# AvishaiBarnoy/genomics-lm

Measured on AMD Instinct MI355X. Metric: codon tokens/sec training step, 12L8H d512 seq1024, higher is better.
Workload: dtype bf16; 1 GPU; TinyGPT 12L8H d512 T1024 V68 train step; model=TinyGPT (genomics-lm src/codonlm), global_batch=32, seq_len=1024, micro_batch_per_gpu=32, parallelism=dp1, sep_mask=True

## Files before the change

### genomics-lm_amd/csrc/gemm.hip

```cpp
#include "common.h"
#include <algorithm>

struct GemmParams {
  int M, N, K, kchunk;
  const void* A; long long lda;
  const void* B; long long ldb;
  void* C; long long ldc; int c_dtype;
  int epi; float alpha;
  const float* bias;
  const float* resid; long long ldr;
  const void* aux; void* aux_out; long long ld_aux;
  uint32_t drop_seed, drop_thr; float drop_scale;
  float* ws; int split;
  int n_valid;
  const float* rope_cos; const float* rope_sin;
  int rope_T, rope_half, rope_G, rope_mul, rope_uqk;
};

__device__ __forceinline__ void epi_apply(const GemmParams& p, int row, int col, float v) {
  const int e = p.epi;
  if (e & CG_EPI_BIAS) v += p.bias[col];
  const long long ai = (long long)row * p.ld_aux + col;
  if (e & CG_EPI_GELU) {
    const float s = (e & CG_EPI_GELU_DERIV) ? dgelu_f(v) : v;
// ... 269 lines not shown
template <bool KC>
__device__ __forceinline__ v8bf frag(const char* img, int rr0, int ks, int lane) {
  if (KC) {
    const int row = rr0 + (lane & 15), ch = ks * 4 + (lane >> 4);
    return *(const v8bf*)(img + kc_off(row, ch));
  } else {
    const int g = lane >> 4, i16 = lane & 15, q = i16 >> 2, pp = i16 & 3;
    const int krow = ks * 32 + 8 * g + q;
    const int ch = (rr0 >> 3) + (pp >> 1);
    const int b0 = mc_off(krow, ch) + 8 * (pp & 1);
    const int b1 = mc_off(krow + 4, ch) + 8 * (pp & 1);
    typedef v4s __attribute__((address_space(3))) * lp4;
    v4s lo = __builtin_amdgcn_ds_read_tr16_b64_v4i16((lp4)(img + b0));
    v4s hi = __builtin_amdgcn_ds_read_tr16_b64_v4i16((lp4)(img + b1));
    v8s r = {lo[0], lo[1], lo[2], lo[3], hi[0], hi[1], hi[2], hi[3]};
    return __builtin_bit_cast(v8bf, r);
  }
}
}

__device__ __forceinline__ void ld8f(const float* p, float v[8]) {
  const float4 a = *(const float4*)p, b = *(const float4*)(p + 4);
  v[0] = a.x; v[1] = a.y; v[2] = a.z; v[3] = a.w; v[4] = b.x; v[5] = b.y; v[6] = b.z; v[7] = b.w;
}
__device__ __forceinline__ void st8f(float* p, const float v[8]) {
  *(float4*)p = make_float4(v[0], v[1], v[2], v[3]);
  *(float4*)(p + 4) = make_float4(v[4], v[5], v[6], v[7]);
}
__device__ __forceinline__ void ld8b(const bf16_t* p, float v[8]) {
  const uint4 u = *(const uint4*)p;
  const uint32_t w[4] = {u.x, u.y, u.z, u.w};
#pragma unroll
  for (int j = 0; j < 4; ++j) {
    v[2 * j] = __uint_as_float(w[j] << 16);
    v[2 * j + 1] = __uint_as_float(w[j] & 0xFFFF0000u);
  }
}
__device__ __forceinline__ void st8b(bf16_t* p, const float v[8]) {
  uint4 u;
  u.x = (uint32_t)f2bf(v[0]) | ((uint32_t)f2bf(v[1]) << 16);
  u.y = (uint32_t)f2bf(v[2]) | ((uint32_t)f2bf(v[3]) << 16);
  u.z = (uint32_t)f2bf(v[4]) | ((uint32_t)f2bf(v[5]) << 16);
  u.w = (uint32_t)f2bf(v[6]) | ((uint32_t)f2bf(v[7]) << 16);
  *(uint4*)p = u;
}

template <int EPI, int CT>
__device__ __forceinline__ void epi_apply8(const GemmParams& p, int row, int col, float v[8]) {
  const int e = EPI >= 0 ? EPI : p.epi;
  const int ct = EPI >= 0 ? CT : p.c_dtype;
  if (e & CG_EPI_BIAS) {
    float bb[8];
    ld8f(p.bias + col, bb);
#pragma unroll
    for (int j = 0; j < 8; ++j) v[j] += bb[j];
  }
  const long long ai = (long long)row * p.ld_aux + col;
  if (e & CG_EPI_GELU) {
    if (e & CG_EPI_GELU_DERIV) {
      float dg[8];
#pragma unroll
      for (int j = 0; j < 8; ++j) v[j] = gelu_fast_d(v[j], dg[j]);
      if (ct == CG_BF16) st8b((bf16_t*)p.aux_out + ai, dg);
      else st8f((float*)p.aux_out + ai, dg);
    } else {
      if (ct == CG_BF16) st8b((bf16_t*)p.aux_out + ai, v);
      else st8f((float*)p.aux_out + ai, v);
#pragma unroll
      for (int j = 0; j < 8; ++j) v[j] = gelu_fast(v[j]);
    }
  }
  if (e & CG_EPI_DGELU) {
    float a[8];
    if (ct == CG_BF16) ld8b((const bf16_t*)p.aux + ai, a);
    else ld8f((const float*)p.aux + ai, a);
    if (e & CG_EPI_GELU_DERIV) {
#pragma unroll
      for (int j = 0; j < 8; ++j) v[j] *= a[j];
    } else {
#pragma unroll
      for (int j = 0; j < 8; ++j) v[j] *= dgelu_fast(a[j]);
    }
  }
  if (e & CG_EPI_DROPOUT) {
#pragma unroll
    for (int j = 0; j < 8; j += 2) {
      const uint32_t h = cg_hash_pair(p.drop_seed, (uint32_t)row, (uint32_t)(col + j) >> 1);
      v[j] = (h & 0xFFFFu) >= p.drop_thr ? v[j] * p.drop_scale : 0.f;
      v[j + 1] = (h >> 16) >= p.drop_thr ? v[j + 1] * p.drop_scale : 0.f;
    }
  }
  if (e & CG_EPI_RESID) {
    float r[8];
    ld8f(p.resid + (long long)row * p.ldr + col, r);
#pragma unroll
    for (int j = 0; j < 8; ++j) v[j] += r[j];
  }
  const long long ci = (long long)row * p.ldc + col;
  if (ct == CG_BF16) {
    st8b((bf16_t*)p.C + ci, v);
  } else {
    float* c = (float*)p.C + ci;
    if (e & CG_EPI_ACCUM) {
      float o[8];
      ld8f(c, o);
#pragma unroll
      for (int j = 0; j < 8; ++j) v[j] += o[j];
    }
    st8f(c, v);
  }
}

__global__ __launch_bounds__(256) void splitk_reduce_vec_kernel(GemmParams p) {
  const long long total8 = (long long)p.M * p.N / 8;
  const long long slab = (long long)p.M * p.N;
  for (long long i = blockIdx.x * 256ll + threadIdx.x; i < total8; i += (long long)gridDim.x * 256) {
    float s[8], t[8];
    ld8f(p.ws + i * 8, s);
    for (int z = 1; z < p.split; ++z) {
      ld8f(p.ws + z * slab + i * 8, t);
#pragma unroll
      for (int j = 0; j < 8; ++j) s[j] += t[j];
    }
    const long long e = i * 8;
    epi_apply8<-1, 0>(p, (int)(e / p.N), (int)(e % p.N), s);
  }
}

namespace bfg {
constexpr int EPI_LD = 68;
constexpr int EPI_BYTES = 4 * 64 * EPI_LD * 4;
constexpr int SMEM = EPI_BYTES > 4 * TILE_BYTES ? EPI_BYTES : 4 * TILE_BYTES;
}

template <bool AK, bool BKC, int EPI, int CT, bool VEC>
__device__ __forceinline__ void gemm_bf16_body(const GemmParams& p, char* smem) {
  using namespace bfg;
#define AS(i) (smem + (i) * TILE_BYTES)
#define BS(i) (smem + (2 + (i)) * TILE_BYTES)
  const int tid = threadIdx.x, wave = tid >> 6, lane = tid & 63;
  const int wm = (wave >> 1) * 64, wn = (wave & 1) * 64;
  const int nwg = gridDim.x * gridDim.y * gridDim.z;
  const int wg = cg_xcd_remap(blockIdx.x + gridDim.x * (blockIdx.y + gridDim.y * blockIdx.z), nwg);
  const int bz = wg / (gridDim.x * gridDim.y), bxy = wg % (gridDim.x * gridDim.y);
  const int m0 = (bxy / gridDim.x) * BM, n0 = (bxy % gridDim.x) * BN;
  const int kbeg = bz * p.kchunk;
  const int kend = min(p.K, kbeg + p.kchunk);
  const bf16_t* A = (const bf16_t*)p.A;
  const bf16_t* B = (const bf16_t*)p.B;

  v4f acc[4][4];
#pragma unroll
  for (int i = 0; i < 4; ++i)
#pragma unroll
    for (int j = 0; j < 4; ++j) acc[i][j] = (v4f){0.f, 0.f, 0.f, 0.f};

  const int nt = (kend - kbeg + BKT - 1) / BKT;
  Stage sa, sb;
  if (nt > 0) {
    stage_load<AK>(sa, A, p.lda, m0, p.M, kbeg, kend, tid);
    stage_load<BKC>(sb, B, p.ldb, n0, p.N, kbeg, kend, tid);
    stage_store<AK>(sa, AS(0), tid);
    stage_store<BKC>(sb, BS(0), tid);
  }
  __syncthreads();
  for (int t = 0; t < nt; ++t) {
    const int cur = t & 1;
    const bool more = (t + 1) < nt;
    if (more) {
      const int kn = kbeg + (t + 1) * BKT;
      stage_load<AK>(sa, A, p.lda, m0, p.M, kn, kend, tid);
      stage_load<BKC>(sb, B, p.ldb, n0, p.N, kn, kend, tid);
    }
#pragma unroll
    for (int ks = 0; ks < 2; ++ks) {
      v8bf af[4], bfr[4];
#pragma unroll
      for (int i = 0; i < 4; ++i) af[i] = frag<AK>(AS(cur), wm + 16 * i, ks, lane);
#pragma unroll
      for (int j = 0; j < 4; ++j) bfr[j] = frag<BKC>(BS(cur), wn + 16 * j, ks, lane);
      __builtin_amdgcn_s_setprio(1);
#pragma unroll
      for (int i = 0; i < 4; ++i)
#pragma unroll
        for (int j = 0; j < 4; ++j)
          acc[i][j] = __builtin_amdgcn_mfma_f32_16x16x32_bf16(af[i], bfr[j], acc[i][j], 0, 0, 0);
      __builtin_amdgcn_s_setprio(0);
    }
    if (more) {
      stage_store<AK>(sa, AS(cur ^ 1), tid);
      stage_store<BKC>(sb, BS(cur ^ 1), tid);
    }
    __syncthreads();
  }
#undef AS
#undef BS
  if (!VEC) {
#pragma unroll
    for (int i = 0; i < 4; ++i)
#pragma unroll
      for (int j = 0; j < 4; ++j)
#pragma unroll
        for (int v = 0; v < 4; ++v) {
          const int row = m0 + wm + 16 * i + 4 * (lane >> 4) + v;
          const int col = n0 + wn + 16 * j + (lane & 15);
          epi_store(p, row, col, acc[i][j][v], bz);
        }
    return;
  }
  float* st = (float*)smem + wave * 64 * EPI_LD;
#pragma unroll
  for (int i = 0; i < 4; ++i)
#pragma unroll
    for (int j = 0; j < 4; ++j)
#pragma unroll
      for (int v = 0; v < 4; ++v) st[(16 * i + 4 * (lane >> 4) + v) * EPI_LD + 16 * j + (lane & 15)] = acc[i][j][v];
  __syncthreads();
#pragma unroll 2
  for (int it = 0; it < 8; ++it) {
    const int c = lane + 64 * it, r = c >> 3, ch = c & 7;
    const int row = m0 + wm + r, col = n0 + wn + ch * 8;
    if (row >= p.M || col >= p.N) continue;
    float v[8];
    ld8f(st + r * EPI_LD + ch * 8, v);
#pragma unroll
    for (int j = 0; j < 8; ++j) v[j] *= p.alpha;
    if (p.split > 1) {
      st8f(p.ws + ((long long)bz * p.M + row) * p.N + col, v);
      continue;
    }
    epi_apply8<EPI, CT>(p, row, col, v);
  }
}

template <bool AK, bool BKC>
__global__ __launch_bounds__(256, 2) void gemm_bf16_kernel(GemmParams p) {
  extern __shared__ __attribute__((aligned(16))) char smem[];
  gemm_bf16_body<AK, BKC, -1, 0, false>(p, smem);
}

template <bool AK, bool BKC, int EPI, int CT>
__global__ __launch_bounds__(256, 2) void gemm_bf16_vec_kernel(GemmParams p) {
  extern __shared__ __attribute__((aligned(16))) char smem[];
  gemm_bf16_body<AK, BKC, EPI, CT, true>(p, smem);
}

#include "gemm_wide.h"
#include "gemm_pers.h"
#include "gemm_lw.h"
#include "gemm_dw.h"

__global__ __launch_bounds__(256) void colsum64_kernel(const void* C, long long ldc, int ct, int M, int N,
                                                       float* __restrict__ part) {
  const int n = blockIdx.x * 256 + threadIdx.x;
  if (n >= N) return;
  const int r0 = blockIdx.y * 64, r1 = min(M, r0 + 64);
  float acc = 0.f;
  for (int r = r0; r < r1; ++r)
    acc += ct == CG_BF16 ? bf2f(((const bf16_t*)C)[(long long)r * ldc + n]) : ((const float*)C)[(long long)r * ldc + n];
  part[(long long)blockIdx.y * N + n] = acc;
}

typedef void (*gemm_kernel_t)(GemmParams);

template <typename K>
static void launch4(K k00, K k01, K k10, K k11, bool ak, bool bk, dim3 g, dim3 b, size_t sh,
                    hipStream_t s, const GemmParams& p) {
  K k = ak ? (bk ? k11 : k10) : (bk ? k01 : k00);
  hipLaunchKernelGGL(k, g, b, sh, s, p);
}

template <template <bool, bool, int, int> class KS>
static gemm_kernel_t pick_spec(bool ak, bool bk, int e, int ct) {
#define SPEC(AK_, BK_, E, T) \
  if (ak == AK_ && bk == BK_ && e == (E) && ct == (T)) return KS<AK_, BK_, (E), (T)>::fn;
  SPEC(true, true, 0, CG_BF16)
  SPEC(true, true, 0, CG_F32)
  SPEC(true, true, CG_EPI_BIAS, CG_BF16)
  SPEC(true, true, CG_EPI_BIAS | CG_EPI_RESID, CG_F32)
  SPEC(true, true, CG_EPI_BIAS | CG_EPI_GELU, CG_BF16)
  SPEC(true, true, CG_EPI_BIAS | CG_EPI_DROPOUT | CG_EPI_RESID, CG_F32)
  SPEC(true, true, CG_EPI_RESID, CG_F32)
  SPEC(true, true, CG_EPI_DROPOUT | CG_EPI_RESID, CG_F32)
  SPEC(true, true, CG_EPI_DGELU, CG_BF16)
  SPEC(true, true, CG_EPI_BIAS | CG_EPI_GELU | CG_EPI_GELU_DERIV, CG_BF16)
  SPEC(true, true, CG_EPI_DGELU | CG_EPI_GELU_DERIV, CG_BF16)
  SPEC(true, false, 0, CG_BF16)
  SPEC(true, false, 0, CG_F32)
  SPEC(true, false, CG_EPI_DGELU, CG_BF16)
  SPEC(false, false, 0, CG_F32)
  SPEC(false, false, CG_EPI_ACCUM, CG_F32)
#undef SPEC
  if (ak) return bk ? KS<true, true, -1, 0>::fn : KS<true, false, -1, 0>::fn;
  return bk ? KS<false, true, -1, 0>::fn : KS<false, false, -1, 0>::fn;
}
template <bool AK, bool BKC, int E, int T>
struct VecK { static constexpr gemm_kernel_t fn = gemm_bf16_vec_kernel<AK, BKC, E, T>; };
template <bool AK, bool BKC, int E, int T>
struct WideK { static constexpr gemm_kernel_t fn = gemm_bf16_wide_kernel<AK, BKC, E, T>; };

static bool lw_auto_for(int e) {
  return e == 0 || e == CG_EPI_BIAS || e == (CG_EPI_BIAS | CG_EPI_GELU) ||
         e == (CG_EPI_BIAS | CG_EPI_GELU | CG_EPI_GELU_DERIV) || e == (CG_EPI_BIAS | CG_EPI_RESID) ||
         e == CG_EPI_RESID || e == CG_EPI_SWIGLU || (e & CG_EPI_ROPE);
}
static gemm_kernel_t pick_pers(int e, int ct, int tile, bool* lw_out) {
  bool lw = tile == CG_TILE_PERS_LW || (tile == CG_TILE_AUTO && lw_auto_for(e));
  if (e == CG_EPI_DSWIGLU) lw = false;
  if (e & CG_EPI_ROPE) {
    if (ct != CG_BF16 || !lw) return nullptr;
    *lw_out = true;
    if (e == (CG_EPI_BIAS | CG_EPI_ROPE)) return gemm_bf16_lw_kernel<CG_EPI_BIAS | CG_EPI_ROPE, CG_BF16>;
    if (e == CG_EPI_ROPE) return gemm_bf16_lw_kernel<CG_EPI_ROPE, CG_BF16>;
    return nullptr;
  }
  *lw_out = lw;
#define PSPEC(E, T) \
  if (e == (E) && ct == (T)) return lw ? gemm_bf16_lw_kernel<(E), (T)> : gemm_bf16_pers_kernel<(E), (T)>;
  PSPEC(0, CG_BF16)
  PSPEC(0, CG_F32)
  PSPEC(CG_EPI_BIAS, CG_BF16)
  PSPEC(CG_EPI_BIAS | CG_EPI_RESID, CG_F32)
  PSPEC(CG_EPI_BIAS | CG_EPI_GELU, CG_BF16)
  PSPEC(CG_EPI_BIAS | CG_EPI_DROPOUT | CG_EPI_RESID, CG_F32)
  PSPEC(CG_EPI_RESID, CG_F32)
  PSPEC(CG_EPI_DROPOUT | CG_EPI_RESID, CG_F32)
  PSPEC(CG_EPI_DGELU, CG_BF16)
  PSPEC(CG_EPI_ACCUM, CG_F32)
  PSPEC(CG_EPI_DGELU | CG_EPI_COLSUM, CG_BF16)
  PSPEC(CG_EPI_BIAS | CG_EPI_GELU | CG_EPI_GELU_DERIV, CG_BF16)
  PSPEC(CG_EPI_DGELU | CG_EPI_GELU_DERIV, CG_BF16)
  PSPEC(CG_EPI_DGELU | CG_EPI_GELU_DERIV | CG_EPI_COLSUM, CG_BF16)
  PSPEC(CG_EPI_COLSUM, CG_BF16)
  PSPEC(CG_EPI_SWIGLU, CG_BF16)
  PSPEC(CG_EPI_DSWIGLU, CG_BF16)
#undef PSPEC
  return nullptr;
}
static int cu_count() {
  static int n[64] = {0};
  int dev = 0;
  (void)hipGetDevice(&dev);
  if (dev < 0 || dev >= 64) dev = 0;
  if (!n[dev]) {
    int v = 0;
    if (hipDeviceGetAttribute(&v, hipDeviceAttributeMultiprocessorCount, dev) != hipSuccess || v <= 0) v = 256;
    n[dev] = v;
  }
  return n[dev];
}
extern "C" int cg_pers_cus(void) { return cu_count(); }
static bool use_pers(const cg_gemm_desc* d, int split) {
  if (split != 1) return false;
  if (d->tile != CG_TILE_AUTO && d->tile != CG_TILE_PERS && d->tile != CG_TILE_PERS_LW) return false;
  if (!d->a_kcontig || !d->b_kcontig) return false;
  if (d->K % bfp::BKT || d->K < 2 * bfp::BKT) return false;
  bool lw = false;
  if (!pick_pers(d->epilogue, d->c_dtype, d->tile, &lw)) return false;
  const long long lim = (long long)bfp::OOR - (1ll << 24);
  const long long es = d->c_dtype == CG_BF16 ? 2 : 4;
  if (((long long)(d->M - 1) * d->lda + d->K) * 2 >= lim) return false;
  if (((long long)(d->N - 1) * d->ldb + d->K) * 2 >= lim) return false;
  if (((long long)(d->M - 1) * d->ldc + d->N) * es >= lim) return false;
  if ((d->epilogue & CG_EPI_RESID) && ((long long)(d->M - 1) * d->ldr + d->N) * 4 >= lim) return false;
  if ((d->epilogue & (CG_EPI_GELU | CG_EPI_DGELU)) && ((long long)(d->M - 1) * d->ld_aux + d->N) * es >= lim)
    return false;
  if ((d->epilogue & (CG_EPI_SWIGLU | CG_EPI_DSWIGLU)) &&
      (((long long)(2 * d->N - 1) * d->ldb + d->K) * 2 >= lim ||
       ((long long)(d->M - 1) * d->ld_aux + 2 * d->N) * 2 >= lim ||
       ((long long)(d->M - 1) * d->ldc + 2 * d->N) * 2 >= lim))
    return false;
  return true;
}

static bool use_wide(const cg_gemm_desc* d, int kchunk, int split) {
  if (d->tile != CG_TILE_AUTO && d->tile != CG_TILE_WIDE) return false;
  if (d->K % bfw::BKT || kchunk % bfw::BKT || d->M < bfw::BM || d->N < bfw::BN) return false;
  if (d->tile == CG_TILE_WIDE) return true;
  if (!d->a_kcontig || !d->b_kcontig) return false;
  const long long tiles = (long long)cg_cdiv(d->M, bfw::BM) * cg_cdiv(d->N, bfw::BN) * split;
  return tiles >= 192;
}

static bool vec_ok(const cg_gemm_desc* d, int split) {
  const int e = d->epilogue;
  if (d->N % 8 || d->ldc % 8 || ((uintptr_t)d->C & 15)) return false;
  if ((e & CG_EPI_BIAS) && ((uintptr_t)d->bias & 15)) return false;
  if ((e & CG_EPI_RESID) && (d->ldr % 8 || ((uintptr_t)d->resid & 15))) return false;
  if ((e & (CG_EPI_GELU | CG_EPI_DGELU)) &&
      (d->ld_aux % 8 || ((uintptr_t)((e & CG_EPI_GELU) ? d->aux_out : d->aux) & 15)))
    return false;
  if (split > 1 && ((uintptr_t)d->workspace & 15)) return false;
  return true;
}

extern "C" int cg_gemm(const cg_gemm_desc* d, void* stream) {
  if (!d || d->M < 0 || d->N < 0 || d->K < 0) return CG_EINVAL;
  if (d->M == 0 || d->N == 0) return CG_OK;
  hipStream_t s = (hipStream_t)stream;
  GemmParams p{};
  p.M = d->M; p.N = d->N; p.K = d->K;
  p.A = d->A; p.lda = d->lda; p.B = d->B; p.ldb = d->ldb;
  p.C = d->C; p.ldc = d->ldc; p.c_dtype = d->c_dtype;
  p.epi = d->epilogue; p.alpha = d->alpha;
  p.bias = d->bias; p.resid = d->resid; p.ldr = d->ldr;
  p.aux = d->aux; p.aux_out = d->aux_out; p.ld_aux = d->ld_aux;
  p.drop_seed = d->drop_seed;
  p.drop_thr = cg_drop_threshold(d->drop_p);
  p.drop_scale = d->drop_p < 1.f ? 1.0f / (1.0f - d->drop_p) : 0.f;
  if ((p.epi & CG_EPI_ACCUM) && p.c_dtype != CG_F32) return CG_EINVAL;
  if ((p.epi & CG_EPI_BIAS) && !p.bias) return CG_EINVAL;
  if ((p.epi & CG_EPI_RESID) && !p.resid) return CG_EINVAL;
  if ((p.epi & CG_EPI_GELU) && !p.aux_out) return CG_EINVAL;
  if ((p.epi & CG_EPI_DGELU) && !p.aux) return CG_EINVAL;
  if ((p.epi & CG_EPI_GELU_DERIV) && !(p.epi & (CG_EPI_GELU | CG_EPI_DGELU))) return CG_EINVAL;
  if ((p.epi & CG_EPI_COLSUM) && (!d->workspace || d->split_k > 1)) return CG_EINVAL;
  if ((p.epi & CG_EPI_COLSUM) && d->ws_bytes < (size_t)cg_cdiv(p.M, 64) * (size_t)p.N * sizeof(float)) return CG_EINVAL;
  const bool swg = (p.epi & (CG_EPI_SWIGLU | CG_EPI_DSWIGLU)) != 0;
  if (swg) {
    if (p.epi != CG_EPI_SWIGLU && p.epi != CG_EPI_DSWIGLU) return CG_EUNSUPPORTED;
    if (d->in_dtype != CG_BF16 || p.c_dtype != CG_BF16 || d->split_k > 1 || !d->a_kcontig || !d->b_kcontig ||
        p.alpha != 1.0f || (p.N & 63) || (p.ldc & 7) || (p.ld_aux & 7) || ((uintptr_t)p.C & 15) ||
        ((uintptr_t)(p.epi == CG_EPI_SWIGLU ? p.aux_out : p.aux) & 15))
      return CG_EUNSUPPORTED;
    if (p.epi == CG_EPI_SWIGLU ? !p.aux_out : !p.aux) return CG_EINVAL;
    p.n_valid = d->n_valid > 0 ? std::min(d->n_valid, p.N) : p.N;
  }
  const bool rope = (p.epi & CG_EPI_ROPE) != 0;
  if (rope) {
    if ((p.epi & ~(CG_EPI_ROPE | CG_EPI_BIAS)) || !d->rope_cos || !d->rope_sin || d->rope_T <= 0) return CG_EINVAL;
    const int hd = d->rope_hd;
    if (d->in_dtype != CG_BF16 || p.c_dtype != CG_BF16 || d->split_k > 1 || hd <= 0 || hd % 16 ||
        d->rope_heads <= 0 || (long long)d->rope_heads * hd > p.N || p.N % 16 || p.N >= 65536 ||
        (((uintptr_t)d->rope_cos | (uintptr_t)d->rope_sin) & 15))
      return CG_EUNSUPPORTED;
    p.rope_cos = d->rope_cos;
    p.rope_sin = d->rope_sin;
    p.rope_T = d->rope_T;
    p.rope_half = hd / 2;
    p.rope_G = hd / 16;
    p.rope_mul = (65536 + p.rope_G - 1) / p.rope_G;
    p.rope_uqk = d->rope_heads * hd / 16;
  }
  if (d->tile < CG_TILE_AUTO || d->tile > CG_TILE_PERS_LW) return CG_EINVAL;
  if (d->tile != CG_TILE_AUTO && d->in_dtype != CG_BF16) return CG_EUNSUPPORTED;
  int split = d->split_k > 1 ? d->split_k : 1;
  const int bkt = d->in_dtype == CG_BF16 ? bfg::BKT : 16;
  if (d->K == 0) split = 1;
  int kchunk = cg_cdiv(cg_cdiv(d->K > 0 ? d->K : 1, split), bkt) * bkt;
  split = cg_cdiv(d->K > 0 ? d->K : 1, kchunk);
  if (split > 1 && (!d->workspace || d->ws_bytes < (size_t)split * (size_t)p.M * (size_t)p.N * sizeof(float)))
    return CG_EINVAL;
  p.kchunk = kchunk; p.split = split; p.ws = d->workspace;
  bool vec = false;
  const bool colsum = (p.epi & CG_EPI_COLSUM) != 0;
  bool colsum_fused = false;

  if (d->in_dtype == CG_F32) {
    p.epi &= ~CG_EPI_COLSUM;
    const bool big = !(d->lda & 3) && !(d->ldb & 3) && !((uintptr_t)d->A & 15) &&
                     !((uintptr_t)d->B & 15) && ((d->a_kcontig || d->b_kcontig) ? !(d->K & 3) : true) &&
                     (d->a_kcontig || !(d->M & 3)) && (d->b_kcontig || !(d->N & 3));
    if (big) {
      launch4(gemm_f32_big_kernel<false, false>, gemm_f32_big_kernel<false, true>, gemm_f32_big_kernel<true, false>,
              gemm_f32_big_kernel<true, true>, d->a_kcontig, d->b_kcontig,
              dim3(cg_cdiv(p.N, f32b::BN), cg_cdiv(p.M, f32b::BM), split), dim3(256), 0, s, p);
    } else {
      dim3 g(cg_cdiv(p.N, 64), cg_cdiv(p.M, 64), split);
      launch4(gemm_f32_kernel<false, false>, gemm_f32_kernel<false, true>, gemm_f32_kernel<true, false>,
              gemm_f32_kernel<true, true>, d->a_kcontig, d->b_kcontig, g, dim3(256), 0, s, p);
    }
  } else if (d->in_dtype == CG_BF16) {
    if ((d->lda & 7) || (d->ldb & 7)) return CG_EUNSUPPORTED;
    if (((uintptr_t)d->A & 15) || ((uintptr_t)d->B & 15)) return CG_EUNSUPPORTED;
    if (d->a_kcontig ? (d->K & 7) : (d->M & 7)) return CG_EUNSUPPORTED;
    if (d->b_kcontig ? (d->K & 7) : (d->N & 7)) return CG_EUNSUPPORTED;
    dim3 g(cg_cdiv(p.N, bfg::BN), cg_cdiv(p.M, bfg::BM), split);
    dim3 blk(256);
    size_t sh = bfg::SMEM;
    vec = vec_ok(d, split);
    gemm_kernel_t k;
    const bool pers = vec && use_pers(d, split);
    if ((swg || rope) && !pers) return CG_EUNSUPPORTED;
    if (!pers) p.epi &= ~CG_EPI_COLSUM;
    const int ke = split > 1 ? 0 : p.epi, kt = split > 1 ? CG_F32 : p.c_dtype;
    if (pers) {
      bool lw = false;
      k = pick_pers(p.epi, p.c_dtype, d->tile, &lw);
      colsum_fused = colsum;
      const int tiles = cg_cdiv(p.N, (p.epi & CG_EPI_SWIGLU) ? bfp::BN / 2 : bfp::BN) * cg_cdiv(p.M, bfp::BM);
      g = dim3(std::min(tiles, d->max_wg > 0 ? d->max_wg : cg_pers_cus()));
      blk = dim3(lw ? bfl::THREADS : bfp::THREADS);
      sh = lw ? bfl::SMEM : bfp::SMEM;
    } else if (vec && use_wide(d, kchunk, split)) {
      k = pick_spec<WideK>(d->a_kcontig, d->b_kcontig, ke, kt);
      g = dim3(cg_cdiv(p.N, bfw::BN) * cg_cdiv(p.M, bfw::BM) * split);
      blk = dim3(bfw::THREADS);
      sh = bfw::SMEM;
    } else if (vec && (d->tile == CG_TILE_AUTO || d->tile == CG_TILE_VEC)) {
      k = pick_spec<VecK>(d->a_kcontig, d->b_kcontig, ke, kt);
    } else if (d->tile != CG_TILE_AUTO && d->tile != CG_TILE_VEC) {
      return CG_EUNSUPPORTED;
    } else {
      k = d->a_kcontig ? (d->b_kcontig ? gemm_bf16_kernel<true, true> : gemm_bf16_kernel<true, false>)
                       : (d->b_kcontig ? gemm_bf16_kernel<false, true> : gemm_bf16_kernel<false, false>);
    }
    cg_func_lds((const void*)k, (int)sh);
    const int pk = pers ? CG_PROBE_GEMM_PERS
                        : d->a_kcontig ? (d->b_kcontig ? CG_PROBE_GEMM_FWD : CG_PROBE_GEMM_DX)
                                       : (d->b_kcontig ? CG_PROBE_NONE : CG_PROBE_GEMM_DW);
    cg_probe_begin(pk, s);
    hipLaunchKernelGGL(k, g, blk, sh, s, p);
    if (cg_probe_kind() == pk) {
      const double M = p.M, N = p.N, K = p.K, ce = p.c_dtype == CG_F32 ? 4.0 : 2.0;
      const bool sw = (p.epi & CG_EPI_SWIGLU) != 0, dsw = (p.epi & CG_EPI_DSWIGLU) != 0;
      const double nb = sw ? 2.0 * N : N;
      double bytes = 2.0 * (M * K + nb * K) + M * N * ce;
      if (p.epi & CG_EPI_BIAS) bytes += 4.0 * N;
      if (p.epi & CG_EPI_RESID) bytes += 4.0 * M * N;
      if (p.epi & (CG_EPI_GELU | CG_EPI_DGELU)) bytes += M * N * ce;
      if (p.epi & CG_EPI_ACCUM) bytes += 4.0 * M * N;
      if (sw) bytes += 2.0 * M * 2.0 * N;
      if (dsw) bytes += 2.0 * M * 2.0 * N + M * N * ce;
      if (p.epi & CG_EPI_COLSUM) bytes += 4.0 * cg_cdiv(p.M, 64) * N;
      cg_probe_end(pk, s, 2.0 * M * nb * K, bytes);
    }
  } else {
    return CG_EUNSUPPORTED;
  }
  CG_LAUNCH_CHECK();
  if (split > 1) {
    const long long total = (long long)p.M * p.N;
    if (vec) {
      int blocks = (int)((total / 8 + 255) / 256);
      if (blocks > 4096) blocks = 4096;
      hipLaunchKernelGGL(splitk_reduce_vec_kernel, dim3(blocks), dim3(256), 0, s, p);
    } else {
      int blocks = (int)((total + 255) / 256);
      if (blocks > 4096) blocks = 4096;
      hipLaunchKernelGGL(splitk_reduce_kernel, dim3(blocks), dim3(256), 0, s, p);
    }
    CG_LAUNCH_CHECK();
  }
  if (colsum && !colsum_fused) {
    hipLaunchKernelGGL(colsum64_kernel, dim3(cg_cdiv(p.N, 256), cg_cdiv(p.M, 64)), dim3(256), 0, s, p.C, p.ldc,
                       p.c_dtype, p.M, p.N, p.ws);
    CG_LAUNCH_CHECK();
  }
  return CG_OK;
}

#ifndef DW_RING_SLOTS
#define DW_RING_SLOTS 5
#endif
static bool dw_tile_code(int bm) { return bm == 128 || bm == 129 || bm == 256 || bm == 512; }
extern "C" int cg_gemm_dw_tiles(int bm, int N_out, int K_out) {
  if (!dw_tile_code(bm)) bm = 128;
  return cg_cdiv(N_out, bm >= 256 ? 256 : 128) * cg_cdiv(K_out, bm == 512 ? 256 : 128);
}
template <int BM, int NS, int BNT = bfd::BN, int BKT = DW_KUNIT>
static int launch_dw(bfd::Params& P, hipStream_t s) {
  using G = bfd::Geo<BM, NS, BNT, BKT>;
  bool cs = false;
  for (int i = 0; i < P.nprod; ++i) cs |= P.p[i].colsum != nullptr;
  auto kern = cs ? gemm_dw_kernel<BM, NS, BNT, true, BKT> : gemm_dw_kernel<BM, NS, BNT, false, BKT>;
  int ntiles = 0;
  for (int i = 0; i < P.nprod; ++i) {
    bfd::Prod& pr = P.p[i];
    pr.tiles_n = cg_cdiv(pr.K_out, BNT);
    pr.tile0 = ntiles;
    ntiles += cg_cdiv(pr.N_out, BM) * pr.tiles_n;
  }
  P.ntiles = ntiles * P.ksplit;
  if (!ntiles) return CG_OK;
  if (P.ksplit > 1) P.kc_steps = dw_kc_steps(P.K, P.ksplit);
  const int grid = std::min(P.ntiles, P.max_wg > 0 ? P.max_wg : cg_pers_cus());
  cg_func_lds((const void*)kern, G::SMEM);
  double flops = 0, bytes = 0;
  for (int i = 0; i < P.nprod; ++i) {
    const bfd::Prod& q = P.p[i];
    flops += 2.0 * q.N_out * (double)q.K_out * P.K;
    bytes += 2.0 * P.K * ((double)q.N_out + q.K_out) + (q.accum ? 8.0 : 4.0) * q.N_out * (double)q.K_out;
  }
  cg_probe_begin(CG_PROBE_GEMM_DW_GROUPED, s);
  hipLaunchKernelGGL(kern, dim3(grid), dim3(G::THREADS), G::SMEM, s, P);
  cg_probe_end(CG_PROBE_GEMM_DW_GROUPED, s, flops, bytes);
  if (P.ksplit > 1) {
    long long most = 0;
    double elems = 0;
    for (int i = 0; i < P.nprod; ++i) {
      most = std::max<long long>(most, (long long)P.p[i].N_out * P.p[i].K_out / 4);
      elems += (double)P.p[i].N_out * P.p[i].K_out;
    }
    cg_probe_begin(CG_PROBE_DW_SLAB, s);
    hipLaunchKernelGGL(dw_slab_reduce_kernel, dim3((unsigned)std::min<long long>(cg_cdiv(most, 256), 512), P.nprod),
                       dim3(256), 0, s, P);
    cg_probe_end(CG_PROBE_DW_SLAB, s, (P.ksplit - 1) * elems, (4.0 * (P.ksplit - 1) + 8.0) * elems);
  }
  CG_LAUNCH_CHECK();
  return CG_OK;
}
extern "C" size_t cg_gemm_dw_grouped_workspace(const cg_dw_group* grp) {
  if (!grp || grp->ksplit <= 1) return 0;
  size_t e = 0;
  for (int i = 0; i < grp->n && i < CG_DW_MAX; ++i)
    if (grp->p[i].N_out > 0 && grp->p[i].K_out > 0) e += (size_t)grp->p[i].N_out * (size_t)grp->p[i].K_out;
  return (size_t)(grp->ksplit - 1) * e * sizeof(float);
}
extern "C" size_t cg_gemm_dw_grouped_workspace(const cg_dw_group* grp);
extern "C" int cg_gemm_dw_grouped(const cg_dw_group* grp, void* stream) {
  if (!grp || grp->n < 0 || grp->n > CG_DW_MAX || grp->K <= 0) return CG_EINVAL;
  bfd::Params P{};
  P.nprod = 0;
  P.K = grp->K;
  const long long lim = (1ll << 31) - (1ll << 24);
  for (int i = 0; i < grp->n; ++i) {
    const cg_dw_product& q = grp->p[i];
    if (q.N_out <= 0 || q.K_out <= 0) continue;
    if (!q.A || !q.B || !q.C) return CG_EINVAL;
    if (q.N_out % 8 || q.K_out % 8 || q.lda % 8 || q.ldb % 8 || q.ldc % 4 || q.lda < q.N_out || q.ldb < q.K_out ||
        q.ldc < q.K_out)
      return CG_EUNSUPPORTED;
    if (((uintptr_t)q.A & 15) || ((uintptr_t)q.B & 15) || ((uintptr_t)q.C & 15)) return CG_EUNSUPPORTED;
    if (((long long)(grp->K - 1) * q.lda + q.N_out) * 2 >= lim || ((long long)(grp->K - 1) * q.ldb + q.K_out) * 2 >= lim)
      return CG_EUNSUPPORTED;
    bfd::Prod& pr = P.p[P.nprod++];
    pr.A = (const bf16_t*)q.A; pr.lda = q.lda;
    pr.B = (const bf16_t*)q.B; pr.ldb = q.ldb;
    pr.C = q.C; pr.ldc = q.ldc;
    pr.N_out = q.N_out; pr.K_out = q.K_out;
    pr.alpha = q.alpha; pr.accum = q.accumulate;
    pr.colsum = q.col_sum;
    if (q.col_sum && grp->ksplit > 1) return CG_EUNSUPPORTED;
  }
  if (!P.nprod) return CG_OK;
  P.ksplit = grp->ksplit > 1 ? grp->ksplit : 1;
  if (P.ksplit > 8) return CG_EUNSUPPORTED;
  if (P.ksplit > 1) {
    if (!grp->workspace || ((uintptr_t)grp->workspace & 15) || grp->ws_bytes < cg_gemm_dw_grouped_workspace(grp))
      return CG_EINVAL;
    P.slab = grp->workspace;
    long long off = 0;
    for (int i = 0; i < P.nprod; ++i) {
      P.slab_off[i] = off;
      off += (long long)P.p[i].N_out * P.p[i].K_out;
    }
    P.slab_stride = off;
  }
  hipStream_t s = (hipStream_t)stream;
  const int bm = grp->tile_m > 0 ? grp->tile_m : 128;
  P.max_wg = grp->max_wg;
  if (bm == 512) return launch_dw<256, DW_RING_SLOTS, 256, 32>(P, s);
  if (bm == 256) return launch_dw<256, 3>(P, s);
  if (bm == 129) return launch_dw<128, 5>(P, s);
  return launch_dw<128, 4>(P, s);
}
```

### genomics-lm_amd/csrc/gemm_lw.h

```cpp
namespace bfl {
constexpr int CWAVES = 8, LWAVES = 4, THREADS = 64 * (CWAVES + LWAVES);
constexpr int A_PIECES = bfw::A_BYTES / 1024, B_PIECES = bfw::B_BYTES / 1024;
constexpr int LA = A_PIECES / LWAVES, LB = B_PIECES / LWAVES;
constexpr int PER_STAGE = LA + LB;
constexpr int SMEM = bfp::SMEM;
}

template <int EPI, int CT>
__global__ __launch_bounds__(bfl::THREADS, 1) void gemm_bf16_lw_kernel(GemmParams p) {
  using namespace bfp;
  constexpr bool SWG = Epi<EPI, CT>::SWG, DSW = Epi<EPI, CT>::DSW;
  constexpr bool RP = (EPI & CG_EPI_ROPE) != 0;
  constexpr int BNO = SWG ? BN / 2 : BN;
  constexpr int ES = CT == CG_BF16 ? 2 : 4;
  auto rope_col = [&](int n) __attribute__((always_inline)) {
    const int U = ((n >> 6) << 2) | ((n >> 3) & 3), c = (n >> 5) & 1, e = n & 7;
    if (U < p.rope_uqk) {
      const int h = (U * p.rope_mul) >> 16;
      return h * 2 * p.rope_half + 8 * (U - h * p.rope_G) + c * p.rope_half + e;
    }
    return 16 * U + 8 * c + e;
  };
  extern __shared__ __attribute__((aligned(16))) char smem[];
  const int tid = threadIdx.x, lane = tid & 63;
  const int wave = __builtin_amdgcn_readfirstlane(tid >> 6);
  const int tiles_n = (p.N + BNO - 1) / BNO, tiles_m = (p.M + BM - 1) / BM;
  const int ntiles = tiles_n * tiles_m;
  const int nblk = gridDim.x;
  const int lb = cg_xcd_remap(blockIdx.x, nblk);
  const int my_tiles = lb < ntiles ? (ntiles - 1 - lb) / nblk + 1 : 0;
  const int nt = p.K / BKT;
  const int S = my_tiles * nt;
  auto tile_org = [&](int k, int& m0, int& n0) __attribute__((always_inline)) {
    const int tile = lb + k * nblk;
    m0 = (tile / tiles_n) * BM;
    n0 = (tile % tiles_n) * BNO;
  };

  if (wave >= bfl::CWAVES) {
    const int L = wave - bfl::CWAVES;
    const __amdgpu_buffer_rsrc_t ra = rsrc(p.A, ((long long)(p.M - 1) * p.lda + p.K) * 2);
    const __amdgpu_buffer_rsrc_t rb = rsrc(p.B, ((long long)((SWG ? 2 : 1) * p.N - 1) * p.ldb + p.K) * 2);
    uint32_t va[bfl::LA], vb[bfl::LB];
#pragma unroll
    for (int j = 0; j < bfl::LA; ++j) va[j] = bfw::src_off<true>((L + bfl::LWAVES * j) * 1024 + 16 * lane, p.lda);
#pragma unroll
    for (int j = 0; j < bfl::LB; ++j) {
      const int pos = (L + bfl::LWAVES * j) * 1024 + 16 * lane;
      vb[j] = SWG ? b_src_off_swg(pos, p.ldb, p.N) : b_src_off(pos, p.ldb);
    }
    uint32_t vcur[bfl::LB], vnext[bfl::LB];
    auto rope_offsets = [&](int k) __attribute__((always_inline)) {
      int m0, n0;
      tile_org(k < my_tiles ? k : 0, m0, n0);
#pragma unroll
      for (int j = 0; j < bfl::LB; ++j) {
        const int pos = (L + bfl::LWAVES * j) * 1024 + 16 * lane;
        const int row = pos >> 7, phys = (pos >> 4) & 7;
        vnext[j] = ((uint32_t)rope_col(n0 + row) * (uint32_t)p.ldb + 8u * (uint32_t)(phys ^ fb(row))) * 2u;
      }
    };
    auto issue = [&](int g) __attribute__((always_inline)) {
      uint32_t ao = OOR, bo = OOR;
      if (g < S) {
        const int k = g / nt, t = g - k * nt;
        int m0, n0;
        tile_org(k, m0, n0);
        ao = (uint32_t)(((long long)m0 * p.lda + t * BKT) * 2);
        if constexpr (RP) {
          bo = (uint32_t)(t * BKT * 2);
          if (t == 0) {
#pragma unroll
            for (int j = 0; j < bfl::LB; ++j) vcur[j] = vnext[j];
          }
        } else {
          bo = (uint32_t)(((long long)n0 * p.ldb + t * BKT) * 2);
        }
      }
      char* st = smem + (g % STAGES) * STAGE_BYTES;
#pragma unroll
      for (int j = 0; j < bfl::LA; ++j) bfw::dma16(ra, st + (L + bfl::LWAVES * j) * 1024, ao + va[j]);
#pragma unroll
      for (int j = 0; j < bfl::LB; ++j)
        bfw::dma16(rb, st + A_BYTES + (L + bfl::LWAVES * j) * 1024, RP ? (bo == OOR ? OOR : bo + vcur[j]) : bo + vb[j]);
      if constexpr (RP) {
        if ((g + 1) % nt == 0) rope_offsets((g + 1) / nt);
      }
    };
    if constexpr (RP) rope_offsets(0);
    issue(0);
    issue(1);
    for (int g = 0; g < S; ++g) {
      wait_vm<bfl::PER_STAGE>();
      __builtin_amdgcn_s_barrier();
      issue(g + 2);
    }
    asm volatile("s_waitcnt vmcnt(0)" ::: "memory");
    return;
  }

  const int wm = (wave >> 1) * 64, wn = (wave & 1) * 64;
  const __amdgpu_buffer_rsrc_t rc = rsrc(p.C, ((long long)(p.M - 1) * p.ldc + (DSW ? 2 : 1) * p.N) * ES);
  const int g4 = lane >> 4, r16 = lane & 15;
  u32x4 xa[4][2], xb[4][2], bq[2][2];
  auto cols_of = [&](int n0, int c) __attribute__((always_inline)) {
    if constexpr (RP) return rope_col(n0 + wn + 32 * c + 8 * g4);
    return SWG ? n0 + (wn >> 1) + 8 * g4 : n0 + wn + 32 * c + 8 * g4;
  };
  auto epi_loads = [&](int k, auto lo_t, auto hi_t, auto bias_t) __attribute__((always_inline)) {
    constexpr int LO = decltype(lo_t)::value, HI = decltype(hi_t)::value;
    int m0, n0;
    tile_org(k, m0, n0);
    if constexpr (decltype(bias_t)::value && (EPI & CG_EPI_BIAS) != 0) {
      const __amdgpu_buffer_rsrc_t rbias = rsrc(p.bias, (long long)p.N * 4);
#pragma unroll
      for (int c = 0; c < 2; ++c) {
        const int cc = cols_of(n0, c);
        const uint32_t o = cc < p.N ? (uint32_t)cc * 4u : OOR;
        bq[c][0] = bld(rbias, o);
        bq[c][1] = bld(rbias, o + 16);
      }
    }
#pragma unroll
    for (int i = LO; i < HI; ++i) {
      const int row = m0 + wm + 16 * i + r16;
      const bool rok = row < p.M;
#pragma unroll
      for (int c = 0; c < 2; ++c) {
        const int cc = cols_of(n0, c);
        const bool ok = rok && cc < p.N;
        if constexpr ((EPI & CG_EPI_RESID) != 0) {
          const __amdgpu_buffer_rsrc_t rr = rsrc(p.resid, ((long long)(p.M - 1) * p.ldr + p.N) * 4);
          const uint32_t o = ok ? (uint32_t)(((long long)row * p.ldr + cc) * 4) : OOR;
          xa[i][c] = bld(rr, o);
          xb[i][c] = bld(rr, o + 16);
        }
        if constexpr ((EPI & CG_EPI_DGELU) != 0) {
          const __amdgpu_buffer_rsrc_t rx = rsrc(p.aux, ((long long)(p.M - 1) * p.ld_aux + p.N) * ES);
          const uint32_t o = ok ? (uint32_t)(((long long)row * p.ld_aux + cc) * ES) : OOR;
          xa[i][c] = bld(rx, o);
          if constexpr (CT != CG_BF16) xb[i][c] = bld(rx, o + 16);
        }
        if constexpr ((EPI & CG_EPI_ACCUM) != 0) {
          const uint32_t o = ok ? (uint32_t)(((long long)row * p.ldc + cc) * ES) : OOR;
          xa[i][c] = bld(rc, o);
          xb[i][c] = bld(rc, o + 16);
        }
        if constexpr (DSW) {
          const __amdgpu_buffer_rsrc_t rx = rsrc(p.aux, ((long long)(p.M - 1) * p.ld_aux + 2 * p.N) * 2);
          const uint32_t o = ok ? (uint32_t)(((long long)row * p.ld_aux + cc) * 2) : OOR;
          xa[i][c] = bld(rx, o);
          xb[i][c] = bld(rx, ok ? o + (uint32_t)p.N * 2u : OOR);
        }
      }
    }
  };

  v4f acc[4][4];
  auto cstep = [&](int g) __attribute__((always_inline)) {
    asm volatile("s_waitcnt lgkmcnt(0)" ::: "memory");
    __builtin_amdgcn_s_barrier();
    __builtin_amdgcn_sched_barrier(0);
    const char* st = smem + (g % STAGES) * STAGE_BYTES;
    const char* as = st;
    const char* bs = st + A_BYTES;
    v8bf af[2][4], bfr[2][4];
#pragma unroll
    for (int i = 0; i < 4; ++i) af[0][i] = bfg::frag<true>(as, wm + 16 * i, 0, lane);
#pragma unroll
    for (int j = 0; j < 4; ++j) bfr[0][j] = bfrag(bs, wn, j, 0, lane);
#pragma unroll
    for (int gr = 0; gr < 8; ++gr) {
      const int i = gr >> 1, j0 = 2 * (gr & 1);
      acc[i][j0] = PMFMA(bfr[0][j0], af[0][i], acc[i][j0], 0, 0, 0);
      acc[i][j0 + 1] = PMFMA(bfr[0][j0 + 1], af[0][i], acc[i][j0 + 1], 0, 0, 0);
      if (gr < 4) af[1][gr] = bfg::frag<true>(as, wm + 16 * gr, 1, lane);
      else bfr[1][gr - 4] = bfrag(bs, wn, gr - 4, 1, lane);
    }
#pragma unroll
    for (int i = 0; i < 4; ++i)
#pragma unroll
      for (int j = 0; j < 4; ++j) acc[i][j] = PMFMA(bfr[1][j], af[1][i], acc[i][j], 0, 0, 0);
    __builtin_amdgcn_sched_group_barrier(0x100, 8, 0);
#pragma unroll
    for (int gr = 0; gr < 8; ++gr) {
      __builtin_amdgcn_sched_group_barrier(0x008, 2, 0);
      __builtin_amdgcn_sched_group_barrier(0x100, 1, 0);
    }
    __builtin_amdgcn_sched_group_barrier(0x008, 16, 0);
  };

  const bool scaled = p.alpha != 1.0f;
  auto epilogue = [&](int k) __attribute__((always_inline)) {
    int m0, n0;
    tile_org(k, m0, n0);
    if (__builtin_expect(scaled, 0)) {
      asm volatile("");
#pragma unroll
      for (int i = 0; i < 4; ++i)
#pragma unroll
        for (int j = 0; j < 4; ++j) acc[i][j] *= p.alpha;
    }
    int col[2];
    uint32_t off_c[4][2];
#pragma unroll
    for (int c = 0; c < 2; ++c) col[c] = cols_of(n0, c);
#pragma unroll
    for (int i = 0; i < 4; ++i) {
      const int row = m0 + wm + 16 * i + r16;
#pragma unroll
      for (int c = 0; c < 2; ++c)
        off_c[i][c] = (row < p.M && col[c] < p.N)
                          ? (uint32_t)(((long long)row * p.ldc + col[c]) * ES)
                          : OOR;
    }
    float bia[2][8];
    if constexpr ((EPI & CG_EPI_BIAS) != 0) {
#pragma unroll
      for (int c = 0; c < 2; ++c) unpack_f32(bq[c][0], bq[c][1], bia[c]);
    }
    float csum[2][8];
    if constexpr ((EPI & CG_EPI_COLSUM) != 0) {
#pragma unroll
      for (int c = 0; c < 2; ++c)
#pragma unroll
        for (int j = 0; j < 8; ++j) csum[c][j] = 0.f;
    }
    if constexpr (SWG) {
      const __amdgpu_buffer_rsrc_t rx = rsrc(p.aux_out, ((long long)(p.M - 1) * p.ld_aux + 2 * p.N) * 2);
#pragma unroll
      for (int i = 0; i < 4; ++i) {
        const int row = m0 + wm + 16 * i + r16;
        float g[8], u[8], sv[8];
#pragma unroll
        for (int h = 0; h < 2; ++h)
#pragma unroll
          for (int q = 0; q < 4; ++q) {
            g[4 * h + q] = acc[i][h][q];
            u[4 * h + q] = acc[i][2 + h][q];
          }
        const bool ok = off_c[i][0] != OOR;
        const uint32_t o = ok ? (uint32_t)(((long long)row * p.ld_aux + col[0]) * 2) : OOR;
        bst_aux(rx, o, pack_bf16(g));
        bst_aux(rx, ok ? o + (uint32_t)p.N * 2u : OOR, pack_bf16(u));
#pragma unroll
        for (int j = 0; j < 8; ++j) sv[j] = col[0] + j < p.n_valid ? silu_f(g[j]) * u[j] : 0.f;
        bst(rc, off_c[i][0], pack_bf16(sv));
      }
      return;
    } else if constexpr (DSW) {
#pragma unroll
      for (int i = 0; i < 4; ++i) {
#pragma unroll
        for (int c = 0; c < 2; ++c) {
          float v[8], g[8], u[8], dg[8], du[8];
#pragma unroll
          for (int h = 0; h < 2; ++h)
#pragma unroll
            for (int q = 0; q < 4; ++q) v[4 * h + q] = acc[i][2 * c + h][q];
          unpack_bf16(xa[i][c], g);
          unpack_bf16(xb[i][c], u);
#pragma unroll
          for (int j = 0; j < 8; ++j) {
            dg[j] = du[j] = 0.f;
            if (col[c] + j < p.n_valid) {
              const float sg = 1.0f / (1.0f + __expf(-g[j]));
              du[j] = v[j] * (g[j] * sg);
              dg[j] = v[j] * u[j] * sg * (1.0f + g[j] * (1.0f - sg));
            }
          }
          bst(rc, off_c[i][c], pack_bf16(dg));
          bst(rc, off_c[i][c] == OOR ? OOR : off_c[i][c] + (uint32_t)p.N * 2u, pack_bf16(du));
        }
      }
      return;
    } else if constexpr (RP) {
      const int U = (((n0 + wn) >> 6) << 2) | g4;
      const bool rot = U < p.rope_uqk;
      const int dim0 = rot ? 8 * (U - ((U * p.rope_mul) >> 16) * p.rope_G) : 0;
      const long long tab_bytes = (long long)p.rope_T * p.rope_half * 4;
      const __amdgpu_buffer_rsrc_t rcs = rsrc(p.rope_cos, tab_bytes), rsn = rsrc(p.rope_sin, tab_bytes);
      u32x4 cq[4][2], sq[4][2];
#pragma unroll
      for (int i = 0; i < 4; ++i) {
        const int row = m0 + wm + 16 * i + r16;
        const uint32_t t = (uint32_t)row % (uint32_t)p.rope_T;
        const uint32_t o = rot ? (t * (uint32_t)p.rope_half + (uint32_t)dim0) * 4u : OOR;
        cq[i][0] = bld(rcs, o);
        cq[i][1] = bld(rcs, o + 16);
        sq[i][0] = bld(rsn, o);
        sq[i][1] = bld(rsn, o + 16);
      }
#pragma unroll
      for (int i = 0; i < 4; ++i) {
        float v0[8], v1[8], cs[8], sn[8];
#pragma unroll
        for (int h = 0; h < 2; ++h)
#pragma unroll
          for (int u = 0; u < 4; ++u) {
            v0[4 * h + u] = acc[i][h][u];
            v1[4 * h + u] = acc[i][2 + h][u];
          }
        if constexpr ((EPI & CG_EPI_BIAS) != 0) {
#pragma unroll
          for (int j = 0; j < 8; ++j) {
            v0[j] += bia[0][j];
            v1[j] += bia[1][j];
          }
        }
        unpack_f32(cq[i][0], cq[i][1], cs);
        unpack_f32(sq[i][0], sq[i][1], sn);
#pragma unroll
        for (int j = 0; j < 8; ++j) {
          const float c = rot ? cs[j] : 1.0f;
          const float y0 = fmaf(v0[j], c, -v1[j] * sn[j]);
          const float y1 = fmaf(v1[j], c, v0[j] * sn[j]);
          v0[j] = y0;
          v1[j] = y1;
        }
        bst(rc, off_c[i][0], pack_bf16(v0));
        bst(rc, off_c[i][1], pack_bf16(v1));
      }
      return;
    }
#pragma unroll
    for (int i = 0; i < 4; ++i) {
      const int row = m0 + wm + 16 * i + r16;
#pragma unroll
      for (int c = 0; c < 2; ++c) {
        float v[8];
#pragma unroll
        for (int h = 0; h < 2; ++h)
#pragma unroll
          for (int u = 0; u < 4; ++u) v[4 * h + u] = acc[i][2 * c + h][u];
        if constexpr ((EPI & CG_EPI_BIAS) != 0) {
#pragma unroll
          for (int j = 0; j < 8; ++j) v[j] += bia[c][j];
        }
        if constexpr ((EPI & CG_EPI_GELU) != 0) {
          const __amdgpu_buffer_rsrc_t rx = rsrc(p.aux_out, ((long long)(p.M - 1) * p.ld_aux + p.N) * ES);
          const uint32_t o = off_c[i][c] == OOR ? OOR : (uint32_t)(((long long)row * p.ld_aux + col[c]) * ES);
          float s[8];
          if constexpr ((EPI & CG_EPI_GELU_DERIV) != 0) {
#pragma unroll
            for (int j = 0; j < 8; ++j) v[j] = gelu_fast_d(v[j], s[j]);
          } else {
#pragma unroll
            for (int j = 0; j < 8; ++j) s[j] = v[j];
          }
          if constexpr (CT == CG_BF16) {
            bst_aux(rx, o, pack_bf16(s));
          } else {
            bst(rx, o, (u32x4){__float_as_uint(s[0]), __float_as_uint(s[1]), __float_as_uint(s[2]), __float_as_uint(s[3])});
            bst(rx, o + 16, (u32x4){__float_as_uint(s[4]), __float_as_uint(s[5]), __float_as_uint(s[6]), __float_as_uint(s[7])});
          }
          if constexpr ((EPI & CG_EPI_GELU_DERIV) == 0) {
#pragma unroll
            for (int j = 0; j < 8; ++j) v[j] = gelu_fast(v[j]);
          }
        }
        if constexpr ((EPI & CG_EPI_DGELU) != 0) {
          float a[8];
          if constexpr (CT == CG_BF16) unpack_bf16(xa[i][c], a);
          else unpack_f32(xa[i][c], xb[i][c], a);
#pragma unroll
          for (int j = 0; j < 8; ++j) v[j] *= (EPI & CG_EPI_GELU_DERIV) ? a[j] : dgelu_fast(a[j]);
        }
        if constexpr ((EPI & CG_EPI_DROPOUT) != 0) {
          const uint32_t rh = cg_row_hash(p.drop_seed, (uint32_t)row);
#pragma unroll
          for (int j = 0; j < 8; j += 2) {
            const uint32_t hsh = cg_pair_mix(rh + ((uint32_t)(col[c] + j) >> 1) * CG_COLK);
            v[j] = (hsh & 0xFFFFu) >= p.drop_thr ? v[j] * p.drop_scale : 0.f;
            v[j + 1] = (hsh >> 16) >= p.drop_thr ? v[j + 1] * p.drop_scale : 0.f;
          }
        }
        if constexpr ((EPI & (CG_EPI_RESID | CG_EPI_ACCUM)) != 0) {
          float r[8];
          unpack_f32(xa[i][c], xb[i][c], r);
#pragma unroll
          for (int j = 0; j < 8; ++j) v[j] += r[j];
        }
        if constexpr ((EPI & CG_EPI_COLSUM) != 0) {
          const float keep = row < p.M ? 1.f : 0.f;
#pragma unroll
          for (int j = 0; j < 8; ++j) csum[c][j] = fmaf(keep, v[j], csum[c][j]);
        }
        if constexpr (CT == CG_BF16) {
          bst(rc, off_c[i][c], pack_bf16(v));
        } else {
          bst(rc, off_c[i][c], (u32x4){__float_as_uint(v[0]), __float_as_uint(v[1]), __float_as_uint(v[2]), __float_as_uint(v[3])});
          bst(rc, off_c[i][c] + 16, (u32x4){__float_as_uint(v[4]), __float_as_uint(v[5]), __float_as_uint(v[6]), __float_as_uint(v[7])});
        }
      }
    }
    if constexpr ((EPI & CG_EPI_COLSUM) != 0) {
#pragma unroll
      for (int c = 0; c < 2; ++c)
#pragma unroll
        for (int j = 0; j < 8; ++j) csum[c][j] = dpp_sum16(csum[c][j]);
      const int prow = (m0 + wm) >> 6;
      const __amdgpu_buffer_rsrc_t rw = rsrc(p.ws, (long long)((p.M + 63) >> 6) * p.N * 4);
#pragma unroll
      for (int c = 0; c < 2; ++c) {
        const uint32_t o = (r16 == 0 && col[c] < p.N) ? (uint32_t)(((long long)prow * p.N + col[c]) * 4) : OOR;
        bst(rw, o, (u32x4){__float_as_uint(csum[c][0]), __float_as_uint(csum[c][1]), __float_as_uint(csum[c][2]),
                           __float_as_uint(csum[c][3])});
        bst(rw, o + 16, (u32x4){__float_as_uint(csum[c][4]), __float_as_uint(csum[c][5]), __float_as_uint(csum[c][6]),
                                __float_as_uint(csum[c][7])});
      }
    }
  };

  constexpr int XW = ((EPI & CG_EPI_RESID) ? 2 : 0) + ((EPI & CG_EPI_DGELU) ? (CT == CG_BF16 ? 1 : 2) : 0) +
                     ((EPI & CG_EPI_ACCUM) ? 2 : 0) + (DSW ? 2 : 0);
  constexpr int HA0 = XW == 0 ? 4 : (32 - ((EPI & CG_EPI_BIAS) ? 16 : 0)) / (8 * XW);
  constexpr int HA = DSW ? 0 : (HA0 > 4 ? 4 : HA0);
  const int ta = nt >= 3 ? nt - 3 : 0;
  int g = 0;
  for (int k = 0; k < my_tiles; ++k) {
#pragma unroll
    for (int i = 0; i < 4; ++i)
#pragma unroll
      for (int j = 0; j < 4; ++j) acc[i][j] = (v4f){0.f, 0.f, 0.f, 0.f};
    for (int t = 0; t < nt; ++t, ++g) {
      cstep(g);
      if (t == ta) {
        __builtin_amdgcn_sched_barrier(0);
        epi_loads(k, std::integral_constant<int, 0>{}, std::integral_constant<int, HA>{}, std::true_type{});
      }
    }
    if constexpr (HA < 4)
      epi_loads(k, std::integral_constant<int, HA>{}, std::integral_constant<int, 4>{}, std::false_type{});
    asm volatile("s_waitcnt vmcnt(0)" ::: "memory");
    __builtin_amdgcn_sched_barrier(0);
    epilogue(k);
  }
}
```

Before: 2.301 million tokens/s.

## Prefetch next-stage LDS fragments mid-step in load-warp GEMM and retime epilogue loads

Restructures the compute-wave main loop of the load-warp persistent GEMM so the barrier and the first-half fragment reads for the next K stage happen in the middle of the current step's second-half MFMAs. This hides LDS read latency behind matrix work instead of stalling at the top of each step. It also changes where epilogue operand loads are issued (late for extra-input epilogues, bias last, halved for accumulate/colsum) to ease register pressure. Finally it routes bias+dropout+residual GEMMs to the LW kernel and allows single-K-tile GEMMs when that kernel is explicitly requested. Risks include higher register use and schedule changes across many epilogue variants.

```diff
diff --git a/genomics-lm_amd/csrc/gemm.hip b/genomics-lm_amd/csrc/gemm.hip
--- a/genomics-lm_amd/csrc/gemm.hip
+++ b/genomics-lm_amd/csrc/gemm.hip
@@ -595,7 +595,8 @@
 static bool lw_auto_for(int e) {
   return e == 0 || e == CG_EPI_BIAS || e == (CG_EPI_BIAS | CG_EPI_GELU) ||
          e == (CG_EPI_BIAS | CG_EPI_GELU | CG_EPI_GELU_DERIV) || e == (CG_EPI_BIAS | CG_EPI_RESID) ||
-         e == CG_EPI_RESID || e == CG_EPI_SWIGLU || (e & CG_EPI_ROPE);
+         e == CG_EPI_RESID || e == (CG_EPI_BIAS | CG_EPI_DROPOUT | CG_EPI_RESID) || e == CG_EPI_SWIGLU ||
+         (e & CG_EPI_ROPE);
 }
 static gemm_kernel_t pick_pers(int e, int ct, int tile, bool* lw_out) {
   bool lw = tile == CG_TILE_PERS_LW || (tile == CG_TILE_AUTO && lw_auto_for(e));
@@ -647,9 +648,10 @@
   if (split != 1) return false;
   if (d->tile != CG_TILE_AUTO && d->tile != CG_TILE_PERS && d->tile != CG_TILE_PERS_LW) return false;
   if (!d->a_kcontig || !d->b_kcontig) return false;
-  if (d->K % bfp::BKT || d->K < 2 * bfp::BKT) return false;
+  if (d->K % bfp::BKT || d->K < bfp::BKT) return false;
   bool lw = false;
   if (!pick_pers(d->epilogue, d->c_dtype, d->tile, &lw)) return false;
+  if (d->K < 2 * bfp::BKT && !(lw && d->tile == CG_TILE_PERS_LW)) return false;
   const long long lim = (long long)bfp::OOR - (1ll << 24);
   const long long es = d->c_dtype == CG_BF16 ? 2 : 4;
   if (((long long)(d->M - 1) * d->lda + d->K) * 2 >= lim) return false;
diff --git a/genomics-lm_amd/csrc/gemm_lw.h b/genomics-lm_amd/csrc/gemm_lw.h
--- a/genomics-lm_amd/csrc/gemm_lw.h
+++ b/genomics-lm_amd/csrc/gemm_lw.h
@@ -157,6 +157,74 @@
   };
 
   v4f acc[4][4];
+#ifndef CG_LW_NO_PREFETCH
+  constexpr int MR = 2;
+  v8bf af[2][4], bfr[2][4];
+  auto read_half0 = [&](int g) __attribute__((always_inline)) {
+    const char* st = smem + (g % STAGES) * STAGE_BYTES;
+#pragma unroll
+    for (int j = 0; j < 4; ++j) bfr[0][j] = bfrag(st + A_BYTES, wn, j, 0, lane);
+#pragma unroll
+    for (int i = 0; i < 4; ++i) af[0][i] = bfg::frag<true>(st, wm + 16 * i, 0, lane);
+  };
+  auto cstep = [&](int g, auto top_tag, auto mid_tag) __attribute__((always_inline)) {
+    constexpr bool MID = decltype(mid_tag)::value;
+    if constexpr (decltype(top_tag)::value) {
+      asm volatile("s_waitcnt lgkmcnt(0)" ::: "memory");
+      __builtin_amdgcn_s_barrier();
+      __builtin_amdgcn_sched_barrier(0);
+      read_half0(g);
+    }
+    const char* st = smem + (g % STAGES) * STAGE_BYTES;
+    const char* as = st;
+    const char* bs = st + A_BYTES;
+#pragma unroll
+    for (int gr = 0; gr < 8; ++gr) {
+      const int i = gr >> 1, j0 = 2 * (gr & 1);
+      acc[i][j0] = PMFMA(bfr[0][j0], af[0][i], acc[i][j0], 0, 0, 0);
+      acc[i][j0 + 1] = PMFMA(bfr[0][j0 + 1], af[0][i], acc[i][j0 + 1], 0, 0, 0);
+      if (gr < 4) af[1][gr] = bfg::frag<true>(as, wm + 16 * gr, 1, lane);
+      else bfr[1][gr - 4] = bfrag(bs, wn, gr - 4, 1, lane);
+    }
+    if constexpr (MID) {
+#pragma unroll
+      for (int i = 0; i < MR; ++i)
+#pragma unroll
+        for (int j = 0; j < 4; ++j) acc[i][j] = PMFMA(bfr[1][j], af[1][i], acc[i][j], 0, 0, 0);
+#pragma unroll
+      for (int gr = 0; gr < 8; ++gr) {
+        __builtin_amdgcn_sched_group_barrier(0x008, 2, 0);
+        __builtin_amdgcn_sched_group_barrier(0x100, 1, 0);
+      }
+      __builtin_amdgcn_sched_group_barrier(0x008, 4 * MR, 0);
+      __builtin_amdgcn_sched_barrier(0);
+      asm volatile("s_waitcnt lgkmcnt(0)" ::: "memory");
+      __builtin_amdgcn_s_barrier();
+      __builtin_amdgcn_sched_barrier(0);
+      read_half0(g + 1);
+#pragma unroll
+      for (int i = MR; i < 4; ++i)
+#pragma unroll
+        for (int j = 0; j < 4; ++j) acc[i][j] = PMFMA(bfr[1][j], af[1][i], acc[i][j], 0, 0, 0);
+#pragma unroll
+      for (int gr = 0; gr < 8; ++gr) {
+        __builtin_amdgcn_sched_group_barrier(0x100, 1, 0);
+        __builtin_amdgcn_sched_group_barrier(0x008, 1, 0);
+      }
+    } else {
+#pragma unroll
+      for (int i = 0; i < 4; ++i)
+#pragma unroll
+        for (int j = 0; j < 4; ++j) acc[i][j] = PMFMA(bfr[1][j], af[1][i], acc[i][j], 0, 0, 0);
+#pragma unroll
+      for (int gr = 0; gr < 8; ++gr) {
+        __builtin_amdgcn_sched_group_barrier(0x008, 2, 0);
+        __builtin_amdgcn_sched_group_barrier(0x100, 1, 0);
+      }
+      __builtin_amdgcn_sched_group_barrier(0x008, 16, 0);
+    }
+  };
+#else
   auto cstep = [&](int g) __attribute__((always_inline)) {
     asm volatile("s_waitcnt lgkmcnt(0)" ::: "memory");
     __builtin_amdgcn_s_barrier();
@@ -189,6 +257,7 @@
     }
     __builtin_amdgcn_sched_group_barrier(0x008, 16, 0);
   };
+#endif
 
   const bool scaled = p.alpha != 1.0f;
   auto epilogue = [&](int k) __attribute__((always_inline)) {
@@ -415,14 +484,45 @@
   constexpr int XW = ((EPI & CG_EPI_RESID) ? 2 : 0) + ((EPI & CG_EPI_DGELU) ? (CT == CG_BF16 ? 1 : 2) : 0) +
                      ((EPI & CG_EPI_ACCUM) ? 2 : 0) + (DSW ? 2 : 0);
   constexpr int HA0 = XW == 0 ? 4 : (32 - ((EPI & CG_EPI_BIAS) ? 16 : 0)) / (8 * XW);
+#ifndef CG_LW_NO_PREFETCH
+  constexpr int HA1 = DSW ? 0 : (HA0 > 4 ? 4 : HA0);
+  constexpr int HA = ((EPI & CG_EPI_ACCUM) || EPI == (CG_EPI_DGELU | CG_EPI_COLSUM)) ? HA1 / 2 : HA1;
+#else
   constexpr int HA = DSW ? 0 : (HA0 > 4 ? 4 : HA0);
+#endif
   const int ta = nt >= 3 ? nt - 3 : 0;
+#ifndef CG_LW_NO_PREFETCH
+  constexpr bool LATE = XW > 0;
+  constexpr bool BIAS_LAST = LATE && HA < 4;
+#endif
   int g = 0;
   for (int k = 0; k < my_tiles; ++k) {
 #pragma unroll
     for (int i = 0; i < 4; ++i)
 #pragma unroll
       for (int j = 0; j < 4; ++j) acc[i][j] = (v4f){0.f, 0.f, 0.f, 0.f};
+#ifndef CG_LW_NO_PREFETCH
+    auto early = [&]() __attribute__((always_inline)) {
+      __builtin_amdgcn_sched_barrier(0);
+      epi_loads(k, std::integral_constant<int, 0>{}, std::integral_constant<int, HA>{}, std::bool_constant<!BIAS_LAST>{});
+    };
+    if (nt == 1) {
+      cstep(g, std::true_type{}, std::false_type{});
+      ++g;
+      early();
+    } else {
+      cstep(g, std::true_type{}, std::true_type{});
+      ++g;
+      if (!LATE && ta == 0) early();
+      for (int t = 1; t < nt - 1; ++t, ++g) {
+        cstep(g, std::false_type{}, std::true_type{});
+        if (!LATE && t == ta) early();
+      }
+      if constexpr (LATE) early();
+      cstep(g, std::false_type{}, std::false_type{});
+      ++g;
+    }
+#else
     for (int t = 0; t < nt; ++t, ++g) {
       cstep(g);
       if (t == ta) {
@@ -430,8 +530,14 @@
         epi_loads(k, std::integral_constant<int, 0>{}, std::integral_constant<int, HA>{}, std::true_type{});
       }
     }
+#endif
+#ifndef CG_LW_NO_PREFETCH
+    if constexpr (HA < 4)
+      epi_loads(k, std::integral_constant<int, HA>{}, std::integral_constant<int, 4>{}, std::bool_constant<BIAS_LAST>{});
+#else
     if constexpr (HA < 4)
       epi_loads(k, std::integral_constant<int, HA>{}, std::integral_constant<int, 4>{}, std::false_type{});
+#endif
     asm volatile("s_waitcnt vmcnt(0)" ::: "memory");
     __builtin_amdgcn_sched_barrier(0);
     epilogue(k);
```

Result: no change. 2.300 million tokens/s (-0.0%).
